# YichengDWu/tinyedm

Hardware: AMD Instinct MI355X
Metric: train imgs/sec CIFAR-10 32x32 bf16 (higher is better)
Workload: dtype bf16; 1 GPU; CIFAR-10 32x32 unconditional EDM2 U-Net (conf/cifar10.yaml, 35.6M params) full training step: diffuse+embed+denoiser fwd/bwd+loss+grad all-reduce+Adam+EMA; per_gpu_batch=128, global_batch=128, parallelism=dp1, conditional=False, step_launch=hipGraph replay, collective=none

## Files before the change

### include/tinyedm_hip.h

```cpp
#ifndef TINYEDM_HIP_H
#define TINYEDM_HIP_H
#ifdef __cplusplus
extern "C" {
#endif

typedef struct ihipStream_t* edm_stream_t;

int edm_version(void);
const char* edm_last_error(void);
int edm_init(int device);
int edm_graph_replay_safe(void);
typedef struct {
  unsigned step, seed_lo, seed_hi, reserved;
  float lr, ema_beta, grad_scale, bc1, bc2sqrt, pad[3];
} edm_step_params;

int edm_conv_igemm(const void* X, const void* Wp, void* Y, const void* R, float alpha, float beta, int B, int H,
                   int W, int Cin, int Cout, int taps, edm_stream_t stream);
int edm_conv_igemm_v2(const void* X, const void* Wp, void* Y, const void* R, float alpha, float beta, int B, int H,
                      int W, int Cin, int Cout, int taps, edm_stream_t stream);
int edm_conv_igemm_v6(const void* X, const void* Wp, void* Y, const void* R, float alpha, float beta, int B, int H,
                      int W, int Cin, int Cout, int taps, edm_stream_t stream);
int edm_conv_igemm_s(const void* X, const void* Wp, void* Y, const void* R, float alpha, float beta, int B, int H,
                     int W, int Cin, int Cout, int taps, edm_stream_t stream);
// ... 82 lines not shown
int edm_attention_fwd(const void* qkv, void* y, int B, int N, int C, int heads, edm_stream_t stream);
int edm_attention_bwd(const void* qkv, const void* y, const void* gy, void* gqkv, int B, int N, int C, int heads,
                      edm_stream_t stream);

int edm_attention_long_supported(int N, int C, int heads);
int edm_attention_long_fwd(const void* qkv, void* y, float* stat, int B, int N, int C, int heads, edm_stream_t stream);
int edm_attention_long_bwd(const void* qkv, const void* y, const void* gy, const float* stat, void* gqkv, float* work,
                           int B, int N, int C, int heads, edm_stream_t stream);

int edm_attention_qkv_supported(int N, int C, int heads);
int edm_attention_qkv_fwd(const void* x, const void* Wqkv, void* y, void* stat, int B, int N, int C, int heads,
                          int heads_per_wg, edm_stream_t stream);
int edm_attention_qkv_bwd(const void* x, const void* y, const void* gout, const void* stat, const void* Wqkv,
                          const void* Wd_out, void* gqkv, float alpha, int B, int N, int C, int heads, int heads_per_wg,
                          edm_stream_t stream);

int edm_pixelnorm_silu_fwd(const void* x, void* xn, void* a, float* dsave, long P, int C, edm_stream_t stream);
int edm_pixelnorm_silu_bwd(const void* xn, const float* dsave, const void* gxn, float gxn_scale, const void* ga,
                           const void* gadd, void* gx, long P, int C, edm_stream_t stream);
int edm_pool_pixelnorm_silu_fwd(const void* x, void* xn, void* a, float* dsave, int B, int Hp, int Wp, int C,
                                edm_stream_t stream);
int edm_pool_pixelnorm_silu_bwd(const void* xn, const float* dsave, const void* gxn, float gxn_scale, const void* ga,
                                const void* gadd, void* gx, int B, int Hp, int Wp, int C, edm_stream_t stream);
int edm_silu_fwd(const void* x, void* a, long n, edm_stream_t stream);
int edm_silu_bwd(const void* x, const void* ga, const void* gextra, float extra_scale, void* gx, long n,
                 edm_stream_t stream);
int edm_axpby(const void* a, float alpha, const void* b, float beta, void* out, long n, edm_stream_t stream);
int edm_mod_silu_drop_fwd(const void* r, const float* lin, long lin_stride, const float* gain, void* a, int B, int HW,
                          int C, float pdrop, unsigned long long seed, unsigned sub, unsigned step, const void* dyn,
                          edm_stream_t stream);
int edm_mod_silu_drop_bwd(const void* r, const float* lin, long lin_stride, const float* gain, const void* ga, void* gr,
                          float* gm, float* glin, long glin_stride, float* ggain, int B, int HW, int C, float pdrop,
                          unsigned long long seed, unsigned sub, unsigned step, const void* dyn, edm_stream_t stream);
int edm_mod_silu_drop_bwd_raw(const void* r, const float* lin, long lin_stride, const float* gain, const void* ga, void* gr,
                              float* gm, long gm_stride, int B, int HW, int C, float pdrop, unsigned long long seed,
                              unsigned sub, unsigned step, const void* dyn, edm_stream_t stream);
int edm_dropout_mask(unsigned char* mask, long n, float pdrop, unsigned long long seed, unsigned sub, unsigned step,
                     edm_stream_t stream);
int edm_pool2(const void* x, void* y, int B, int Hout, int Wout, int C, float scale, edm_stream_t stream);
int edm_up2(const void* x, const void* add, void* y, int B, int Hout, int Wout, int C, float scale, edm_stream_t stream);
int edm_up2_silu(const void* x, void* y, void* a, int B, int Hout, int Wout, int C, edm_stream_t stream);
int edm_reduce_hw(const void* x, long x_stride, const void* y, long y_stride, float* out, int B, int HW, int C,
                  float scale, edm_stream_t stream);
int edm_scalelong_fwd(const float* mean, const float* W1h, const float* W2h, float* gate, float* z1save, int B, int C,
                      int R, edm_stream_t stream);
int edm_scalelong_bwd(const float* mean, const float* W1h, const float* W2h, const float* gate, const float* z1save,
// ... 321 lines not shown
```

### tinyedm_amd/_lib.py

```python
import ctypes
import os

_HERE = os.path.dirname(os.path.abspath(__file__))
LIB_PATH = os.environ.get("EDM_LIB_PATH") or os.path.join(_HERE, "libtinyedm_hip.so")

P, I, L, F = ctypes.c_void_p, ctypes.c_int, ctypes.c_long, ctypes.c_float
U, U64 = ctypes.c_uint, ctypes.c_ulonglong
D = ctypes.c_double

SIGNATURES = {
    "edm_version": [],
    "edm_last_error": [],
    "edm_init": [I],
    "edm_graph_replay_safe": [],
    "edm_pixelnorm_silu_fwd": [P, P, P, P, L, I, P],
    "edm_pixelnorm_silu_bwd": [P, P, P, F, P, P, P, L, I, P],
    "edm_pool_pixelnorm_silu_fwd": [P, P, P, P, I, I, I, I, P],
    "edm_pool_pixelnorm_silu_bwd": [P, P, P, F, P, P, P, I, I, I, I, P],
    "edm_up2_silu": [P, P, P, I, I, I, I, P],
    "edm_silu_fwd": [P, P, L, P],
    "edm_silu_bwd": [P, P, P, F, P, L, P],
    "edm_axpby": [P, F, P, F, P, L, P],
    "edm_mod_silu_drop_fwd": [P, P, L, P, P, I, I, I, F, U64, U, U, P, P],
    "edm_mod_silu_drop_bwd": [P, P, L, P, P, P, P, P, L, P, I, I, I, F, U64, U, U, P, P],
    "edm_mod_silu_drop_bwd_raw": [P, P, L, P, P, P, P, L, I, I, I, F, U64, U, U, P, P],
    "edm_dropout_mask": [P, L, F, U64, U, U, P],
    "edm_pool2": [P, P, I, I, I, I, F, P],
    "edm_up2": [P, P, P, I, I, I, I, F, P],
    "edm_reduce_hw": [P, L, P, L, P, I, I, I, F, P],
    "edm_scalelong_fwd": [P, P, P, P, P, I, I, I, P],
    "edm_scalelong_bwd": [P, P, P, P, P, P, P, P, P, I, I, I, P],
    "edm_skip_gate_fwd": [P, P, P, P, P, P, I, I, I, I, P],
    "edm_skip_gate_bwd": [P, L, I, P, P, P, P, P, P, P, P, P, P, I, I, I, I, P],
    "edm_skip_gate_wgrad_multi": [P, I, P, P, I, P],
    "edm_skip_gate_wgrad_multi_table_bytes": [],
    "edm_skip_gate_fwd_multi": [P, I, P, P, I, P],
    "edm_skip_gate_fwd_multi_table_bytes": [],
    "edm_skip_gate_bwd_multi": [P, I, P, P, I, P],
    "edm_skip_half_bwd_multi": [P, I, P, P, I, P],
    "edm_skip_gate_bwd_multi_table_bytes": [],
    "edm_concat_gate_fwd": [P, P, P, P, P, I, I, I, I, P],
# ... 255 lines not shown
```

### tinyedm_amd/csrc/elementwise.hip

```cpp
#include "common.h"
#include <stdarg.h>
#include <stdio.h>

static thread_local char g_err[512] = "";
extern "C" void edm_set_error(const char* fmt, ...) {
  va_list ap;
  va_start(ap, fmt);
  vsnprintf(g_err, sizeof(g_err), fmt, ap);
  va_end(ap);
}
extern "C" const char* edm_last_error() { return g_err; }
extern "C" int edm_version() { return 1; }

static inline int cdiv(long a, long b) { return (int)((a + b - 1) / b); }
static inline int grid_for(long work, int block, int cap = 256 * 16) {
  long g = (work + block - 1) / block;
  if (g > cap) g = cap;
  if (g < 1) g = 1;
  return (int)g;
}

template <int LPP, bool POOL = false>
__global__ __launch_bounds__(256) void k_pnorm_silu_fwd(const bf16* __restrict__ x, bf16* __restrict__ xn,
                                                          bf16* __restrict__ a, float* __restrict__ dsave, int P,
                                                          int C, int Hp = 0, int Wp = 0) {
// ... 34 lines not shown
      }
    }
    ss = group_sum<LPP>(ss);
    const float d = NORM_EPS + sqrtf(ss) * rsC;
    const float inv = 1.0f / d;
#pragma unroll
    for (int it = 0; it < 2; ++it) {
      const int c8 = lig + it * LPP;
      if (pv && c8 < CL) {
        float o[8], s[8];
#pragma unroll
        for (int i = 0; i < 8; ++i) {
          o[i] = (float)(bf16)(v[it][i] * inv);
          s[i] = mp_silu_b(o[i]);
        }
        store8(xn + p * C + c8 * 8, o);
        store8(a + p * C + c8 * 8, s);
      }
    }
    if (pv && lig == 0) dsave[p] = d;
  }
}

template <int LPP, bool UP = false>
__global__ __launch_bounds__(256) void k_pnorm_silu_bwd(const bf16* __restrict__ xn, const float* __restrict__ dsave,
                                                          const bf16* __restrict__ gxn, float gs,
                                                          const bf16* __restrict__ ga, const bf16* __restrict__ gadd,
                                                          bf16* __restrict__ gx, int P, int C, int Hp = 0, int Wp = 0) {
  constexpr int GPW = 64 / LPP;
  const int lane = threadIdx.x & 63, wave = threadIdx.x >> 6;
  const int lig = lane % LPP, grp = lane / LPP;
  const int CL = C >> 3;
  const long stride = (long)gridDim.x * 4 * GPW;
  for (long p0 = ((long)blockIdx.x * 4 + wave) * GPW; p0 < P; p0 += stride) {
    const long p = p0 + grp;
    const bool pv = p < P;
    float y[2][8], g[2][8];
    float dot = 0.f;
#pragma unroll
    for (int it = 0; it < 2; ++it) {
      const int c8 = lig + it * LPP;
      if (pv && c8 < CL) {
        load8(xn + p * C + c8 * 8, y[it]);
        float t[8];
        if (gxn) {
          load8(gxn + p * C + c8 * 8, t);
#pragma unroll
          for (int i = 0; i < 8; ++i) g[it][i] = gs * t[i];
        } else {
#pragma unroll
          for (int i = 0; i < 8; ++i) g[it][i] = 0.f;
// ... 14 lines not shown
    float inv = 1.0f / d;
#pragma unroll
    for (int it = 0; it < 2; ++it) {
      const int c8 = lig + it * LPP;
      if (pv && c8 < CL) {
        float o[8];
#pragma unroll
        for (int i = 0; i < 8; ++i) o[i] = (g[it][i] - y[it][i] * coef) * inv;
        if constexpr (UP) {
          const int w = (int)(p % Wp);
          const long t2 = p / Wp;
          const int h = (int)(t2 % Hp);
          const long b = t2 / Hp;
          const long e0 = ((b * 2 * Hp + 2 * h) * 2 * Wp + 2 * w) * C + c8 * 8;
          const long row = (long)2 * Wp * C;
#pragma unroll
          for (int i = 0; i < 8; ++i) o[i] = 0.25f * (float)(bf16)o[i];
#pragma unroll
          for (int q = 0; q < 4; ++q) {
            const long e = e0 + (q >> 1) * row + (q & 1) * C;
            float r[8];
#pragma unroll
            for (int i = 0; i < 8; ++i) r[i] = o[i];
            if (gadd) {
              float t[8];
              load8(gadd + e, t);
#pragma unroll
              for (int i = 0; i < 8; ++i) r[i] += t[i];
            }
            store8(gx + e, r);
          }
          continue;
        }
        if (gadd) {
          float t[8];
          load8(gadd + p * C + c8 * 8, t);
#pragma unroll
          for (int i = 0; i < 8; ++i) o[i] += t[i];
        }
        store8(gx + p * C + c8 * 8, o);
      }
    }
  }
}

static int pick_lpp(int C) {
  int cl = C / 8;
  return cl <= 16 ? 16 : (cl <= 32 ? 32 : 64);
}

extern "C" int edm_pixelnorm_silu_fwd(const void* x, void* xn, void* a, float* dsave, long P, int C,
                                      hipStream_t st) {
  EDM_REQUIRE(P > 0 && P < (1L << 31) && C > 0 && C % 8 == 0 && C <= 1024, "pixelnorm_silu_fwd: bad P=%ld C=%d", P, C);
  int lpp = pick_lpp(C);
  int gpw = 64 / lpp;
  int grid = grid_for(P, 4 * gpw);
#define L(N) hipLaunchKernelGGL(k_pnorm_silu_fwd<N>, dim3(grid), dim3(256), 0, st, (const bf16*)x, (bf16*)xn, (bf16*)a, dsave, (int)P, C)
  if (lpp == 16) L(16); else if (lpp == 32) L(32); else L(64);
#undef L
  EDM_CHECK_LAUNCH("pixelnorm_silu_fwd");
  return EDM_OK;
}
// ... 5 lines not shown
  const long P = (long)B * Hp * Wp;
  int lpp = pick_lpp(C);
  int gpw = 64 / lpp;
  int grid = grid_for(P, 4 * gpw);
#define L(N) hipLaunchKernelGGL((k_pnorm_silu_fwd<N, true>), dim3(grid), dim3(256), 0, st, (const bf16*)x, (bf16*)xn, (bf16*)a, dsave, (int)P, C, Hp, Wp)
  if (lpp == 16) L(16); else if (lpp == 32) L(32); else L(64);
#undef L
  EDM_CHECK_LAUNCH("pool_pixelnorm_silu_fwd");
  return EDM_OK;
}
extern "C" int edm_pool_pixelnorm_silu_bwd(const void* xn, const float* dsave, const void* gxn, float gxn_scale,
                                           const void* ga, const void* gadd, void* gx, int B, int Hp, int Wp, int C,
                                           hipStream_t st) {
  EDM_REQUIRE(xn && dsave && gx && B > 0 && Hp > 0 && Wp > 0 && C > 0 && C % 8 == 0 && C <= 1024 &&
                  (long)B * Hp * Wp < (1L << 31), "pool_pixelnorm_silu_bwd: bad args");
  const long P = (long)B * Hp * Wp;
  int lpp = pick_lpp(C);
  int gpw = 64 / lpp;
  int grid = grid_for(P, 4 * gpw);
#define L(N) hipLaunchKernelGGL((k_pnorm_silu_bwd<N, true>), dim3(grid), dim3(256), 0, st, (const bf16*)xn, dsave, (const bf16*)gxn, gxn_scale, (const bf16*)ga, (const bf16*)gadd, (bf16*)gx, (int)P, C, Hp, Wp)
  if (lpp == 16) L(16); else if (lpp == 32) L(32); else L(64);
#undef L
  EDM_CHECK_LAUNCH("pool_pixelnorm_silu_bwd");
  return EDM_OK;
}

extern "C" int edm_pixelnorm_silu_bwd(const void* xn, const float* dsave, const void* gxn, float gxn_scale,
                                      const void* ga, const void* gadd, void* gx, long P, int C, hipStream_t st) {
  EDM_REQUIRE(P > 0 && P < (1L << 31) && C > 0 && C % 8 == 0 && C <= 1024, "pixelnorm_silu_bwd: bad P=%ld C=%d", P, C);
  int lpp = pick_lpp(C);
  int gpw = 64 / lpp;
  int grid = grid_for(P, 4 * gpw);
#define L(N) hipLaunchKernelGGL(k_pnorm_silu_bwd<N>, dim3(grid), dim3(256), 0, st, (const bf16*)xn, dsave, (const bf16*)gxn, gxn_scale, (const bf16*)ga, (const bf16*)gadd, (bf16*)gx, (int)P, C)
  if (lpp == 16) L(16); else if (lpp == 32) L(32); else L(64);
#undef L
  EDM_CHECK_LAUNCH("pixelnorm_silu_bwd");
  return EDM_OK;
}

__global__ void k_silu_fwd(const bf16* __restrict__ x, bf16* __restrict__ a, long n8) {
  for (long i = (long)blockIdx.x * blockDim.x + threadIdx.x; i < n8; i += (long)gridDim.x * blockDim.x) {
    float v[8];
    load8(x + i * 8, v);
#pragma unroll
    for (int j = 0; j < 8; ++j) v[j] = mp_silu_b(v[j]);
    store8(a + i * 8, v);
// ... 1371 lines not shown
```

### tinyedm_amd/networks.py

```python
from __future__ import annotations

import contextlib
import math
import os
from typing import Optional

import numpy as np
import torch
import torch.nn as nn
from torch import Tensor

from . import ops

bf16, f32 = torch.bfloat16, torch.float32


class _Rng:
    seed: int = 42
    step: int = 0
    dyn = None


rng = _Rng()

# ... 81 lines not shown
            if len(pend) >= FIN_GROUP:
                _flush_fin(key)
            _queue_backward_end(w.device)
            return None
        g = ops.wgrad_finish(slabs, w.data, self._taps(), I, perm=self._perm, scale=scale)
        return g.view_as(w)


WGRAD_STREAM = os.environ.get("EDM_WGRAD_STREAM", "1") != "0"
W3_GROUP = max(0, min(ops.W3_MAX_LAYERS, int(os.environ.get("EDM_W3_GROUP", "16"))))
W3_TAIL = max(0, int(os.environ.get("EDM_W3_TAIL", "0")))
_w3_seen = {}
_w3_total = {}
W3_MAXPIX = int(os.environ.get("EDM_W3_MAXPIX", str(1 << 18)))
FIN_GROUP = 40
W1_GROUP = max(0, min(16, int(os.environ.get("EDM_W1_GROUP", "16"))))
_w1_pending = {}
_bwd_end_queued = set()
MOD_DEFER_UNFUSED = os.environ.get("EDM_MOD_DEFER_UNFUSED", "1") != "0"
SG_MULTI = os.environ.get("EDM_SG_MULTI", "1") != "0"
SG_HALVES = os.environ.get("EDM_SG_HALVES", "1") != "0"
SG_BWD_MULTI = os.environ.get("EDM_SG_BWD_MULTI", "1") != "0"
SG_DEFER = os.environ.get("EDM_SG_DEFER", "1") != "0"
_sg_pending = {}
_w3_pending = {}
TAIL_LOWRANK = os.environ.get("EDM_TAIL_LOWRANK", "1") != "0"
_tail_slot = {}
TAIL_FWD = os.environ.get("EDM_TAIL_FWD", "1") != "0"
_tail_fwd_slot = {}
_fin_pending = {}


def _run_on_side(device, fn, tensors=()):
    if WGRAD_STREAM:
        side = ops.side_stream(device)
        side.wait_stream(torch.cuda.current_stream())
        with torch.cuda.stream(side):
            fn()
        for t in tensors:
            t.record_stream(side)
    else:
        fn()


class FusedOptPass:

# ... 63 lines not shown
    dev = items[0][1].device
    args = [(slabs, w.data, w.grad, perm, taps, I, scale, True) for slabs, w, perm, taps, I, scale in items]
    _run_on_side(dev, lambda: ops.wgrad_finish_multi(args), [a[0] for a in args])
    for _, w, *_rest in items:
        w._edm_deferred = False
        for hook in getattr(w, "_edm_hooks", ()):
            hook(w)


def _flush_sg(key):
    items = _sg_pending.pop(key, None)
    if not items:
        return
    outs = ops.skip_gate_wgrad_multi([(ws, mean, R) for _, ws, mean, R in items])
    for (sl, _, _, _), (gw1h, gw2h) in zip(items, outs):
        sl.layer1.finish_grad(gw1h.view(1, 1, *gw1h.shape))
        sl.layer2.finish_grad(gw2h.view(1, 1, *gw2h.shape))


def _backward_end(key):
    _bwd_end_queued.discard(key)
    _tail_slot.pop(key, None)
    _tail_fwd_slot.pop(key, None)
    if key in _w3_seen:
        _w3_total[key] = _w3_seen.pop(key)
    _flush_sg(key)
    _flush_w3(key)
    _flush_fin(key)
    if WGRAD_STREAM:
        torch.cuda.current_stream(key).wait_stream(ops.side_stream(key))


def _queue_backward_end(device):
    key = torch.device(device).index
    if key in _bwd_end_queued:
        return
    try:
        torch.autograd.Variable._execution_engine.queue_callback(lambda: _backward_end(key))
        _bwd_end_queued.add(key)
    except RuntimeError:
        _backward_end(key)


def reset_backward_state():
    _tail_slot.clear()
    _tail_fwd_slot.clear()
    if _bwd_end_queued or _w3_pending or _fin_pending or _w1_pending or _sg_pending:
        _bwd_end_queued.clear()
        for items in _sg_pending.values():
            for sl, *_rest in items:
                sl.layer1.weight._edm_deferred = sl.layer2.weight._edm_deferred = False
        _sg_pending.clear()
        for items in _w1_pending.values():
            for m, _, _, _ in items:
                m.weight._edm_deferred = False
        _w1_pending.clear()
        for items in _fin_pending.values():
            for _, w, *_rest in items:
                w._edm_deferred = False
        _fin_pending.clear()
        for items in _w3_pending.values():
            for m, _, _, _ in items:
                m.weight._edm_deferred = False
        _w3_pending.clear()
        _w3_seen.clear()
        if WGRAD_STREAM:
            for s in ops.side_streams():
                torch.cuda.current_stream(s.device).wait_stream(s)

# ... 608 lines not shown
                gqkv = ops.attention_bwd(qkv, y, gy, mod.num_heads)
        gw_out = _wgrad(mod.out_conv, y, gout, 1, b)
        gx = ops.conv_igemm(gqkv, wd_qkv, 1, residual=gout, alpha=1.0, beta=a)
        gw_qkv = _wgrad(mod.qkv_conv, x, gqkv, 1)
        return gx, gw_qkv, gw_out, None, None, None


class _ResBlockFn(torch.autograd.Function):

    @staticmethod
    def forward(ctx, u, emb, w1x1, w1, w2, wemb, gain, blk, lin_view, glin_view, token, s_pre=None, alias=False,
                gm_view=None, skip=None, w_sl1=None, w_sl2=None, pre=None, dest=None, pool=False, gate_pre=None, tail=0):
        enc = blk.is_encoder
        ctx.set_materialize_grads(False)
        has1 = w1x1 is not None
        taps = 9
        wf1, wd1, _ = blk.conv_3x3_1.packs()
        wf2, wd2, _ = blk.conv_3x3_2.packs()
        batched = lin_view is not None
        weh = None if batched else blk.embed.packs()[2]
        wf11 = wd11 = None
        tail_fwd = False
        ctx.has_skip = skip is not None
        if skip is not None:
            sl = blk.cat_factor
            ctx.sgb = None
            if gate_pre is not None:
                mean, gate, z1, w1h, w2h, ctx.sgb, halves = gate_pre
            else:
                w1h, w2h = sl.layer1.packs()[2], sl.layer2.packs()[2]
                mean, gate, z1 = ops.skip_gate_fwd(skip, w1h, w2h)
            ctx.Ci = u.shape[-1]
            if pre is not None and pre[0].shape[-1] == u.shape[-1] + skip.shape[-1] and pre[0].data_ptr() == u.data_ptr():
                cat, s_pre = pre
                if not (gate_pre is not None and halves == cat.data_ptr()):
                    ops.skip_half_fwd(skip, gate, cat, s_pre)
            else:
                cat, s_pre = ops.concat_gate_fwd(u.contiguous(), skip, gate, True)
            u = cat
            ctx.skip_saved = (skip, mean, gate, z1, w1h, w2h)
        ctx.pool = bool(pool)
        if enc and pool:
            assert not has1
            xres, s, dsave = ops.pool_pixelnorm_silu_fwd(u)
        elif enc:
            x = u
            if has1:
                wf11, wd11, _ = blk.conv_1x1.packs()
                x = ops.conv_igemm(u, wf11, 1)
# ... 108 lines not shown
            ggain = None
            if not deferred and not only:
                for hook in getattr(gp, "_edm_hooks", ()):
                    hook(gp)
        if tfwd is not None:
            gw2 = _wgrad_lowrank(blk.conv_3x3_2, a2, tail[0], tail[1], b, G=tfwd[0])
        elif tail is not None:
            gw2 = _wgrad_lowrank(blk.conv_3x3_2, a2, tail[0], tail[1], b)
        else:
            gw2 = _wgrad(blk.conv_3x3_2, a2, gout, 9, b)
        gwemb = gemb = gtoken = None
        if ctx.batched:
            gtoken = ops.zeros_f32((1,), gout.device) if (ctx.has_token and not only) else None
        elif only:
            pass
        else:
            dweh = ops.linear_wgrad(glin, emb)
            gwemb = blk.embed.finish_grad(dweh.view(1, 1, *dweh.shape))
            gemb = ops.linear_dgrad(glin, weh) if ctx.needs_input_grad[1] else None
        fuse = ops.FUSE_MOD and ops.IGEMM_VERSION == 0 and not enc
        gs = None if fuse else ops.conv_igemm(gr1, wd1, 9)
        gw1 = _wgrad(blk.conv_3x3_1, s, gr1, 9)
        gw11 = None
        if enc and ctx.pool:
            gu = ops.pool_pixelnorm_silu_bwd(xn, dsave, gout, a, gs, gadd=g_alias)
            g_alias = None
        elif enc:
            gx = ops.pixelnorm_silu_bwd(xn, dsave, gout, a, gs, gadd=None if has1 else g_alias)
            if has1:
                gw11 = _wgrad(blk.conv_1x1, u, gx, 1)
                gu = ops.conv_igemm(gx, wd11, 1, residual=g_alias, alpha=1.0, beta=1.0 if g_alias is not None else 0.0)
            else:
                gu = gx
            g_alias = None
        else:
            if tfwd is not None:
                t = ops.conv3x3_silubwd(gr1, wd1, u) if fuse else ops.silu_bwd(u, gs)
                gu, gcs = ops.lowrank_gcat_add(tail[0], tfwd[2], a, t, ctx.Ci if ctx.has_skip else None)
                if has1:
                    gw11 = _wgrad_lowrank(blk.conv_1x1, None, None, tail[1], a, G=tfwd[1])
            elif has1:
                t = ops.conv3x3_silubwd(gr1, wd1, u) if fuse else ops.silu_bwd(u, gs)
                if ctx.has_skip:
                    Ci = ctx.Ci
                    B_, H_, W_, Ct = u.shape
                    gu = torch.empty(B_, H_, W_, Ci, device=u.device, dtype=bf16)
                    gcs = torch.empty(B_, H_, W_, Ct - Ci, device=u.device, dtype=bf16)
                    ops.conv_igemm(gout, wd11, 1, residual=t, alpha=a, beta=1.0, split=(Ci, gu, gcs))
                else:
                    gu = ops.conv_igemm(gout, wd11, 1, residual=t, alpha=a, beta=1.0)
                    gcs = None
                gw11 = _wgrad(blk.conv_1x1, u, gout, 1, a)
            else:
                gu = ops.conv3x3_silubwd(gr1, wd1, u, gout, a) if fuse else ops.silu_bwd(u, gs, gout, a)
                gcs = None
        gskip = gwsl1 = gwsl2 = None
        if ctx.has_skip:
            skip, mean, gate, z1, w1h, w2h = ctx.skip_saved
            Ci = ctx.Ci
            sl = blk.cat_factor
            wsl = (sl.layer1.weight, sl.layer2.weight)
            defer = SG_DEFER and all(w.grad is not None and getattr(w, "_edm_direct", False) for w in wsl)
            sgb = getattr(ctx, "sgb", None)
            queued = False
            if only:
                if gcs is None:
                    gmean, _ws = ops.skip_gate_bwd(gu, Ci, skip, mean, w1h, w2h, gate, z1, defer_wgrad=True)
                    gu, gskip = ops.concat_gate_bwd(gu, gate, gmean, Ci)
                elif defer and sgb is not None and SG_BWD_MULTI:
                    gskip = torch.empty_like(gcs)
                    sgb.pending.append((gcs, skip, w1h, w2h, gate, z1, gskip, sl, mean))
                else:
                    gmean, _ws = ops.skip_gate_bwd(gcs, 0, skip, mean, w1h, w2h, gate, z1, defer_wgrad=True)
                    gskip = ops.skip_half_bwd(gcs, gate, gmean)
            elif gcs is None:
                gmean, *gws = ops.skip_gate_bwd(gu, Ci, skip, mean, w1h, w2h, gate, z1, defer_wgrad=defer)
                gu, gskip = ops.concat_gate_bwd(gu, gate, gmean, Ci)
            elif defer and sgb is not None and SG_BWD_MULTI:
                gskip = torch.empty_like(gcs)
                sgb.pending.append((gcs, skip, w1h, w2h, gate, z1, gskip, sl, mean))
                queued = True
            else:
                gmean, *gws = ops.skip_gate_bwd(gcs, 0, skip, mean, w1h, w2h, gate, z1, defer_wgrad=defer)
                gskip = ops.skip_half_bwd(gcs, gate, gmean)
            if only:
                pass
            elif defer:
                if not queued:
                    _sg_pending.setdefault(wsl[0].device.index, []).append((sl, gws[0], mean, w1h.shape[0]))
                wsl[0]._edm_deferred = wsl[1]._edm_deferred = True
                _queue_backward_end(wsl[0].device)
            else:
                gw1h, gw2h = gws
                gwsl1 = sl.layer1.finish_grad(gw1h.view(1, 1, *gw1h.shape))
                gwsl2 = sl.layer2.finish_grad(gw2h.view(1, 1, *gw2h.shape))
            if sgb is not None:
                sgb.arrived += 1
                if sgb.arrived == sgb.expected:
                    sgb.flush()
        if g_alias is not None:
            gu = ops.axpby(gu, 1.0, g_alias, 1.0)
        return (gu, gemb, gw11, gw1, gw2, gwemb, ggain, None, None, None, gtoken, None, None, None, gskip, gwsl1, gwsl2,
                None, None, None, None, None)


_rng_sub_counter = [0]


class _BlockBase(nn.Module):
    is_encoder = True

    def _common(self, out_channels, embedding_dim, attention, num_heads, dropout_rate):
        self.conv_3x3_2 = Conv2d(out_channels, out_channels, 3)
        self.dropout = nn.Dropout(dropout_rate)
        self.attention = CosineAttention(out_channels, num_heads) if attention else nn.Identity()
        self.embed = Linear(embedding_dim, out_channels)
        self.embed.weight._edm_late = True
        self.gain = nn.Parameter(torch.ones(()))
        self._tail_last = False
# ... 93 lines not shown


def _tag(x: Tensor) -> Tensor:
    x._edm_nhwc = True
    return x


class EncoderBlock(_BlockBase):
    is_encoder = True

    def __init__(self, in_channels: int, out_channels: int, embedding_dim: int, down: bool, attention: bool,
                 num_heads: int = 4, dropout_rate: float = 0.0, add_factor: float = 0.3):
        super().__init__()
        self.dropout_rate = dropout_rate
        self.add_factor = add_factor
        self.resample = DownSample() if down else nn.Identity()
        self.conv_1x1 = Conv2d(in_channels, out_channels, 1) if in_channels != out_channels else nn.Identity()
        self.conv_3x3_1 = Conv2d(out_channels, out_channels, 3)
        self._common(out_channels, embedding_dim, attention, num_heads, dropout_rate)

    def forward(self, input: Tensor, embedding: Tensor, _lin=None, _alias: bool = False, _dest=None):
        x, conv = _as_nhwc(input)
        ualias = None
        emb = None if _lin is not None else _emb32(embedding, x.shape[0])
        if (isinstance(self.resample, DownSample) and FUSE_RESAMPLE and not isinstance(self.conv_1x1, Conv2d)
                and x.shape[-1] <= 1024 and x.shape[1] % 2 == 0 and x.shape[2] % 2 == 0):
            out = self._res(x, emb, _lin, alias=_alias, pool=True, dest=_dest)
            if _alias:
                out, ualias = out
        else:
            if isinstance(self.resample, DownSample):
                if _alias:
                    x, ualias = _ResampleFn.apply(x, False, True)
                else:
                    x = _ResampleFn.apply(x, False)
            if _alias and ualias is None:
                out, ualias = self._res(x, emb, _lin, alias=True, dest=_dest)
            else:
                out = self._res(x, emb, _lin, dest=_dest)
        if conv:
            out = ops.nhwc_bf16_to_nchw(out).to(input.dtype)
        else:
            cat_pre = getattr(out, "_edm_cat", None)
            out = _tag(out)
            if cat_pre is not None:
                out._edm_cat = cat_pre
        return (out, _tag(ualias)) if _alias else out

    def forward_f32(self, x: Tensor, lin: Tensor, want=None):
        pairs = _split_ok(self.conv_3x3_1)
        if (F32_FUSE_OUT and isinstance(self.resample, DownSample) and not isinstance(self.conv_1x1, Conv2d)
                and x.shape[-1] <= 1024):
            xn, s = ops.f32_pool_pixelnorm_silu(x, pairs=pairs)
        else:
            if isinstance(self.resample, DownSample):
                x = ops.f32_pool2(x)
            if isinstance(self.conv_1x1, Conv2d):
                x = _conv_f32(self.conv_1x1, x, 1)
            xn, s = ops.f32_pixelnorm_silu(x, pairs=pairs)
        return _res_f32(self, xn, s, lin, want)


class DecoderBlock(_BlockBase):
    is_encoder = False

    def __init__(self, in_channels: int, out_channels: int, embedding_dim: int, up: bool, attention: bool,
                 num_heads: int = 4, skip_channels: int = 0, dropout_rate: float = 0.0, add_factor: float = 0.3):
        super().__init__()
        self.add_factor = add_factor
# ... 591 lines not shown
        B = noisy.shape[0]
        sig = sigma.detach().float().flatten().contiguous()
        emb = _emb32(embedding, B)

        blocks = self._res_blocks()
        lin_all, glin_all, token, gm_all = _EmbedAllFn.apply(emb, self, *[b.embed.weight for b in blocks])
        lins, off = {}, 0
        for k, b in enumerate(blocks):
            C = b.embed.weight.shape[0]
            lins[b] = (lin_all[:, off:off + C], glin_all[:, off:off + C], token if k == 0 else None,
                       None if gm_all is None else gm_all[:, off:off + C])
            off += C

        link = [] if (torch.is_grad_enabled() and noisy.requires_grad) else None
        x = _ConvInFn.apply(noisy, sig, self.conv_in.weight, self, link)
        skips = []
        dec = list(zip(self.decoder_blocks, self.skip_connections))
        enc = list(self.encoder_blocks)
        for k, block in enumerate(enc):
            dest = None
            if k + 1 == len(enc) and dec and not dec[0][1]:
                dest = self._silu_dest(block, dec[0][0], x, 1, down=isinstance(block.resample, DownSample))
            x, x_in = block(_tag(x), None, _lin=lins[block], _alias=True, _dest=dest)
            skips.append(x_in)
        skips.append(x)
        dests = _decoder_dests_impl(dec, skips, x) if FUSE_CAT and SKIP_GATE_FUSED else {}
        gates = self._decoder_gates(dec, skips, dests) if SG_MULTI else {}
        tail_co = self._tail_fwd_co()
        for i, (block, has_skip) in enumerate(dec):
            skip = skips.pop() if has_skip else None
            dest = dests.get(i)
            if dest is not None:
                pass
            elif i + 1 < len(dec):
                dest = self._silu_dest(block, dec[i + 1][0], x, 2 if isinstance(block.resample, UpSample) else 1)
            xin = _tag(x)
            cat_pre = getattr(x, "_edm_cat", None)
            if cat_pre is not None:
                xin._edm_cat = cat_pre
            last = {"_tail": tail_co} if (tail_co and i + 1 == len(dec)) else {}
            x = block(xin, None, _tag(skip) if has_skip else None, _lin=lins[block], _dest=dest, _gate=gates.get(block), **last)
        D = self._conv_out_of(x, noisy, sig, link)
        if self.training:
            rng.step += 1
        return D.to(noisy_image.dtype)


class _SgbPass:

    def __init__(self, expected: int):
        self.expected, self.arrived, self.pending = expected, 0, []

    def flush(self):
        items, self.pending = self.pending, []
        self.arrived = 0
        if not items:
            return
        by_c = {}
        for it in items:
            by_c.setdefault(it[1].shape[-1], []).append(it)
        halves = []
        for group in by_c.values():
            for k0 in range(0, len(group), 32):
                part = group[k0:k0 + 32]
                res = ops.skip_gate_bwd_multi([(gcs, 0, skip, w1h, w2h, gate, z1) + ((gskip,) if SG_HALVES else ())
                                               for gcs, skip, w1h, w2h, gate, z1, gskip, _, _ in part])
                for (gcs, skip, w1h, w2h, gate, z1, gskip, sl, mean), (gmean, ws) in zip(part, res):
                    if not SG_HALVES:
                        halves.append((gcs, gate, gmean, gskip))
                    if _DGRAD_ONLY[0]:
                        continue
                    _sg_pending.setdefault(sl.layer1.weight.device.index, []).append((sl, ws, mean, w1h.shape[0]))
        for k0 in range(0, len(halves), 32):
            ops.skip_half_bwd_multi(halves[k0:k0 + 32])


def _decoder_dests_impl(dec, skips, x):
    out = {}
    st = list(skips)
    h, w = x.shape[1], x.shape[2]
    for i, (block, has_skip) in enumerate(dec):
        if has_skip:
            st.pop()
        if isinstance(block.resample, UpSample):
            h, w = 2 * h, 2 * w
        if i + 1 < len(dec) and dec[i + 1][1]:
            nxt = dec[i + 1][0]
            if not isinstance(nxt.resample, UpSample) and isinstance(nxt.conv_1x1, Conv2d):
                Ct = block.conv_3x3_2.weight.shape[0] + st[-1].shape[-1]
                out[i] = (torch.empty(x.shape[0], h, w, Ct, device=x.device, dtype=bf16),
                          torch.empty(x.shape[0], h, w, Ct, device=x.device, dtype=bf16))
# ... 49 lines not shown
```

### tinyedm_amd/ops.py

```python
import contextlib
import ctypes
import functools
import math
import os
import types
from typing import NamedTuple, Optional

import numpy as np
import torch

from . import _lib

bf16, f32 = torch.bfloat16, torch.float32

PROFILE = None


class _prof:
    def __init__(self, name, flops, nbytes):
        self.name, self.flops, self.nbytes = name, flops, nbytes

    def __enter__(self):
        if PROFILE is not None:
            self.s = torch.cuda.Event(enable_timing=True)
# ... 281 lines not shown
    return t.shape


def pixelnorm_silu_fwd(x):
    B, H, W, C = _nhwc(x, "x")
    xn, a = torch.empty_like(x), torch.empty_like(x)
    d = torch.empty(B * H * W, device=x.device, dtype=f32)
    _lib.call("edm_pixelnorm_silu_fwd", _p(x), _p(xn), _p(a), _p(d), B * H * W, C, _stream())
    return xn, a, d


def pixelnorm_silu_bwd(xn, d, gxn, gxn_scale, ga, gadd=None):
    B, H, W, C = _nhwc(xn, "xn")
    _chk(d, f32, "d", (B * H * W,))
    if gxn is not None:
        _chk(gxn, bf16, "gxn", xn.shape)
    if ga is not None:
        _chk(ga, bf16, "ga", xn.shape)
    if gadd is not None:
        _chk(gadd, bf16, "gadd", xn.shape)
    gx = torch.empty_like(xn)
    _lib.call("edm_pixelnorm_silu_bwd", _p(xn), _p(d), _p(gxn), float(gxn_scale), _p(ga), _p(gadd), _p(gx), B * H * W, C,
              _stream())
    return gx


def pool_pixelnorm_silu_fwd(x):
    B, H, W, C = _nhwc(x, "x")
    if H % 2 or W % 2 or C > 1024:
        raise ValueError("pool_pixelnorm_silu_fwd: H, W even and C <= 1024 required")
    xn = torch.empty(B, H // 2, W // 2, C, device=x.device, dtype=bf16)
    a = torch.empty_like(xn)
    d = torch.empty(B * (H // 2) * (W // 2), device=x.device, dtype=f32)
    _lib.call("edm_pool_pixelnorm_silu_fwd", _p(x), _p(xn), _p(a), _p(d), B, H // 2, W // 2, C, _stream())
    return xn, a, d


def pool_pixelnorm_silu_bwd(xn, d, gxn, gxn_scale, ga, gadd=None):
    B, H, W, C = _nhwc(xn, "xn")
    _chk(d, f32, "d", (B * H * W,))
    if gxn is not None:
        _chk(gxn, bf16, "gxn", xn.shape)
    if ga is not None:
        _chk(ga, bf16, "ga", xn.shape)
    if gadd is not None:
        _chk(gadd, bf16, "gadd", (B, 2 * H, 2 * W, C))
# ... 3009 lines not shown
```

### tinyedm_amd/vjp.py

```python
from __future__ import annotations

import torch

from . import networks

__all__ = ["input_vjp", "open_input_vjp"]


def _bf16_only(den) -> None:
    if getattr(den, "eval_dtype", "bf16") != "bf16":
        raise ValueError(f"input_vjp: the denoiser evaluates in {den.eval_dtype!r}, a forward-only path; the backward exists "
                         "on the bf16 path: call set_eval_dtype(\"bf16\") (generate: --network_dtype bf16)")


def _check_inputs(x, sigma) -> None:
    if not isinstance(x, torch.Tensor) or not x.dtype.is_floating_point or x.dim() != 4:
        raise ValueError("input_vjp: x must be a floating-point [B, C, H, W] tensor")
    if not x.is_cuda:
        raise ValueError(f"input_vjp: x is on {x.device}; the library's networks run on the GPU only")
    if not isinstance(sigma, torch.Tensor) or sigma.device != x.device:
        raise ValueError(f"input_vjp: sigma must be a tensor on {x.device}")


def _library_parts(model):
# ... 35 lines not shown
            else:
                if not isinstance(labels_or_embedding, torch.Tensor):
                    raise ValueError("input_vjp: a Denoiser takes the embedding tensor as its fourth argument")
                emb = labels_or_embedding
            emb = emb.detach()
        prev, networks._DGRAD_ONLY[0] = networks._DGRAD_ONLY[0], True
        try:
            with torch.enable_grad():
                xr = x.detach().float().contiguous().requires_grad_()
                D = den(xr, sigma.detach(), emb)
        finally:
            networks._DGRAD_ONLY[0] = prev
    finally:
        owner.train(was_training)

    def pullback(cotangent):
        _check_cotangent(cotangent, D)
        prev, networks._DGRAD_ONLY[0] = networks._DGRAD_ONLY[0], True
        try:
            (g,) = torch.autograd.grad(D, xr, cotangent.detach().float().contiguous())
        finally:
            networks._DGRAD_ONLY[0] = prev
            networks._tail_slot.pop(dev, None)
        return g
    return D.detach(), pullback


def _check_cotangent(cotangent, D) -> None:
    if not isinstance(cotangent, torch.Tensor) or not cotangent.dtype.is_floating_point:
        raise ValueError("input_vjp: cotangent must be a floating-point tensor")
    if tuple(cotangent.shape) != tuple(D.shape):
        raise ValueError(f"input_vjp: cotangent must have D's shape {tuple(D.shape)}, got {tuple(cotangent.shape)}")
    if cotangent.device != D.device:
        raise ValueError(f"input_vjp: cotangent is on {cotangent.device}, D on {D.device}")


def input_vjp(model, x, sigma, labels_or_embedding=None, cotangent=None):
    if cotangent is None:
        raise ValueError("input_vjp: cotangent is required (the vector of the vector-Jacobian product)")
    D, pullback = open_input_vjp(model, x, sigma, labels_or_embedding)
    return D, pullback(cotangent)
```

Baseline: 10370 img/s.

## Fold factored skip-gate gradient into encoder pixelnorm-SiLU backward

In the batched skip-gate backward, the dense skip gradient (gcs*gate + gmean/HW) is no longer materialised. The decoder instead records the concat-gradient slice, gate and gmean, and the matching encoder block's pixelnorm-SiLU backward (plain and pooled variants) recomputes that term on the fly while adding it to its output. This removes a full-size bf16 write and read of the skip gradient per skip connection. In exchange it adds cross-block bookkeeping keyed on tensor pointers, an optional bf16 rounding to match the old numerics, and new error paths for when a backward pass ends partway through the decoder.

```diff
diff --git a/include/tinyedm_hip.h b/include/tinyedm_hip.h
--- a/include/tinyedm_hip.h
+++ b/include/tinyedm_hip.h
@@ -128,6 +128,12 @@
                                 edm_stream_t stream);
 int edm_pool_pixelnorm_silu_bwd(const void* xn, const float* dsave, const void* gxn, float gxn_scale, const void* ga,
                                 const void* gadd, void* gx, int B, int Hp, int Wp, int C, edm_stream_t stream);
+int edm_pixelnorm_silu_bwd_fskip(const void* xn, const float* dsave, const void* gxn, float gxn_scale, const void* ga,
+                                 const void* gcat, long gcat_stride, const float* gate, const float* gmean, int HW,
+                                 int round_bf16, void* gx, long P, int C, edm_stream_t stream);
+int edm_pool_pixelnorm_silu_bwd_fskip(const void* xn, const float* dsave, const void* gxn, float gxn_scale, const void* ga,
+                                      const void* gcat, long gcat_stride, const float* gate, const float* gmean, int HW,
+                                      int round_bf16, void* gx, int B, int Hp, int Wp, int C, edm_stream_t stream);
 int edm_silu_fwd(const void* x, void* a, long n, edm_stream_t stream);
 int edm_silu_bwd(const void* x, const void* ga, const void* gextra, float extra_scale, void* gx, long n,
                  edm_stream_t stream);
diff --git a/tinyedm_amd/_lib.py b/tinyedm_amd/_lib.py
--- a/tinyedm_amd/_lib.py
+++ b/tinyedm_amd/_lib.py
@@ -17,6 +17,8 @@
     "edm_pixelnorm_silu_bwd": [P, P, P, F, P, P, P, L, I, P],
     "edm_pool_pixelnorm_silu_fwd": [P, P, P, P, I, I, I, I, P],
     "edm_pool_pixelnorm_silu_bwd": [P, P, P, F, P, P, P, I, I, I, I, P],
+    "edm_pixelnorm_silu_bwd_fskip": [P, P, P, F, P, P, L, P, P, I, I, P, L, I, P],
+    "edm_pool_pixelnorm_silu_bwd_fskip": [P, P, P, F, P, P, L, P, P, I, I, P, I, I, I, I, P],
     "edm_up2_silu": [P, P, P, I, I, I, I, P],
     "edm_silu_fwd": [P, P, L, P],
     "edm_silu_bwd": [P, P, P, F, P, L, P],
diff --git a/tinyedm_amd/csrc/elementwise.hip b/tinyedm_amd/csrc/elementwise.hip
--- a/tinyedm_amd/csrc/elementwise.hip
+++ b/tinyedm_amd/csrc/elementwise.hip
@@ -1,6 +1,7 @@
 #include "common.h"
 #include <stdarg.h>
 #include <stdio.h>
+#include <type_traits>
 
 static thread_local char g_err[512] = "";
 extern "C" void edm_set_error(const char* fmt, ...) {
@@ -81,11 +82,54 @@
   }
 }
 
-template <int LPP, bool UP = false>
+struct FSkip {
+  long gs;
+  const float* gate;
+  const float* gmean;
+  int HW;
+  float inv_hw;
+  int round_bf16;
+};
+template <bool FS, class Fs>
+__device__ __forceinline__ int fskip_sample(long p, const Fs& fs) {
+  if constexpr (FS) return (int)p / fs.HW;
+  else return 0;
+}
+template <bool FS, class Fs>
+__device__ __forceinline__ void fskip_add8(float* o, const bf16* __restrict__ gadd, long pix, long b, long plain_off,
+                                           int c, int C, const Fs& fs) {
+  float t[8];
+  if constexpr (FS) {
+    load8(gadd + pix * fs.gs + c, t);
+    const float4* gp = reinterpret_cast<const float4*>(fs.gate + b * C + c);
+    const float4* mp = reinterpret_cast<const float4*>(fs.gmean + b * C + c);
+    const float4 g0 = gp[0], g1 = gp[1], m0 = mp[0], m1 = mp[1];
+    const float gt[8] = {g0.x, g0.y, g0.z, g0.w, g1.x, g1.y, g1.z, g1.w};
+    const float mn[8] = {m0.x, m0.y, m0.z, m0.w, m1.x, m1.y, m1.z, m1.w};
+#pragma unroll
+    for (int i = 0; i < 8; ++i) t[i] = __builtin_fmaf(t[i], gt[i], mn[i] * fs.inv_hw);
+    if (fs.round_bf16) {
+#pragma unroll
+      for (int i = 0; i < 8; ++i) t[i] = (float)(bf16)t[i];
+    }
+#pragma unroll
+    for (int i = 0; i < 8; ++i) {
+      asm volatile("" : "+v"(o[i]));
+      o[i] += t[i];
+    }
+  } else {
+    load8(gadd + plain_off, t);
+#pragma unroll
+    for (int i = 0; i < 8; ++i) o[i] += t[i];
+  }
+}
+struct NoFSkip {};
+template <int LPP, bool UP = false, bool FS = false>
 __global__ __launch_bounds__(256) void k_pnorm_silu_bwd(const bf16* __restrict__ xn, const float* __restrict__ dsave,
                                                           const bf16* __restrict__ gxn, float gs,
                                                           const bf16* __restrict__ ga, const bf16* __restrict__ gadd,
-                                                          bf16* __restrict__ gx, int P, int C, int Hp = 0, int Wp = 0) {
+                                                          bf16* __restrict__ gx, int P, int C, int Hp = 0, int Wp = 0,
+                                                          std::conditional_t<FS, FSkip, NoFSkip> fs = {}) {
   constexpr int GPW = 64 / LPP;
   const int lane = threadIdx.x & 63, wave = threadIdx.x >> 6;
   const int lig = lane % LPP, grp = lane / LPP;
@@ -146,22 +190,13 @@
             float r[8];
 #pragma unroll
             for (int i = 0; i < 8; ++i) r[i] = o[i];
-            if (gadd) {
-              float t[8];
-              load8(gadd + e, t);
-#pragma unroll
-              for (int i = 0; i < 8; ++i) r[i] += t[i];
-            }
+            if (FS || gadd)
+              fskip_add8<FS>(r, gadd, (b * 2 * Hp + 2 * h + (q >> 1)) * 2 * Wp + 2 * w + (q & 1), b, e, c8 * 8, C, fs);
             store8(gx + e, r);
           }
           continue;
         }
-        if (gadd) {
-          float t[8];
-          load8(gadd + p * C + c8 * 8, t);
-#pragma unroll
-          for (int i = 0; i < 8; ++i) o[i] += t[i];
-        }
+        if (FS || gadd) fskip_add8<FS>(o, gadd, p, fskip_sample<FS>(p, fs), p * C + c8 * 8, c8 * 8, C, fs);
         store8(gx + p * C + c8 * 8, o);
       }
     }
@@ -213,6 +248,57 @@
   if (lpp == 16) L(16); else if (lpp == 32) L(32); else L(64);
 #undef L
   EDM_CHECK_LAUNCH("pool_pixelnorm_silu_bwd");
+  return EDM_OK;
+}
+
+static int fskip_args(const char* who, const void* gcat, long gs, const float* gate, const float* gmean, int HW,
+                      int round_bf16, long pix, int C, FSkip* fs) {
+  EDM_REQUIRE(gcat && gate && gmean, "%s: null pointer", who);
+  EDM_REQUIRE(HW > 0 && pix % HW == 0, "%s: %ld pixels are no whole samples of HW=%d", who, pix, HW);
+  EDM_REQUIRE(gs >= C && gs % 8 == 0 && ((uintptr_t)gcat & 15) == 0, "%s: gcat rows (stride %ld) must be 16-byte aligned", who, gs);
+  EDM_REQUIRE((((uintptr_t)gate | (uintptr_t)gmean) & 15) == 0, "%s: gate / gmean must be 16-byte aligned", who);
+  fs->gs = gs;
+  fs->gate = gate;
+  fs->gmean = gmean;
+  fs->HW = HW;
+  fs->inv_hw = 1.0f / (float)HW;
+  fs->round_bf16 = round_bf16 != 0;
+  return EDM_OK;
+}
+extern "C" int edm_pixelnorm_silu_bwd_fskip(const void* xn, const float* dsave, const void* gxn, float gxn_scale,
+                                            const void* ga, const void* gcat, long gcat_stride, const float* gate,
+                                            const float* gmean, int HW, int round_bf16, void* gx, long P, int C,
+                                            hipStream_t st) {
+  EDM_REQUIRE(xn && dsave && gx && P > 0 && P < (1L << 31) && C > 0 && C % 8 == 0 && C <= 1024,
+              "pixelnorm_silu_bwd_fskip: bad P=%ld C=%d", P, C);
+  FSkip fs;
+  if (int rc = fskip_args("pixelnorm_silu_bwd_fskip", gcat, gcat_stride, gate, gmean, HW, round_bf16, P, C, &fs)) return rc;
+  int lpp = pick_lpp(C);
+  int gpw = 64 / lpp;
+  int grid = grid_for(P, 4 * gpw);
+#define L(N) hipLaunchKernelGGL((k_pnorm_silu_bwd<N, false, true>), dim3(grid), dim3(256), 0, st, (const bf16*)xn, dsave, (const bf16*)gxn, gxn_scale, (const bf16*)ga, (const bf16*)gcat, (bf16*)gx, (int)P, C, 0, 0, fs)
+  if (lpp == 16) L(16); else if (lpp == 32) L(32); else L(64);
+#undef L
+  EDM_CHECK_LAUNCH("pixelnorm_silu_bwd_fskip");
+  return EDM_OK;
+}
+extern "C" int edm_pool_pixelnorm_silu_bwd_fskip(const void* xn, const float* dsave, const void* gxn, float gxn_scale,
+                                                 const void* ga, const void* gcat, long gcat_stride, const float* gate,
+                                                 const float* gmean, int HW, int round_bf16, void* gx, int B, int Hp,
+                                                 int Wp, int C, hipStream_t st) {
+  EDM_REQUIRE(xn && dsave && gx && B > 0 && Hp > 0 && Wp > 0 && C > 0 && C % 8 == 0 && C <= 1024 &&
+                  (long)B * Hp * Wp < (1L << 29), "pool_pixelnorm_silu_bwd_fskip: bad args");
+  EDM_REQUIRE((long)HW == 4L * Hp * Wp, "pool_pixelnorm_silu_bwd_fskip: HW=%d is not the skip's 4 Hp Wp", HW);
+  const long P = (long)B * Hp * Wp;
+  FSkip fs;
+  if (int rc = fskip_args("pool_pixelnorm_silu_bwd_fskip", gcat, gcat_stride, gate, gmean, HW, round_bf16, 4 * P, C, &fs)) return rc;
+  int lpp = pick_lpp(C);
+  int gpw = 64 / lpp;
+  int grid = grid_for(P, 4 * gpw);
+#define L(N) hipLaunchKernelGGL((k_pnorm_silu_bwd<N, true, true>), dim3(grid), dim3(256), 0, st, (const bf16*)xn, dsave, (const bf16*)gxn, gxn_scale, (const bf16*)ga, (const bf16*)gcat, (bf16*)gx, (int)P, C, Hp, Wp, fs)
+  if (lpp == 16) L(16); else if (lpp == 32) L(32); else L(64);
+#undef L
+  EDM_CHECK_LAUNCH("pool_pixelnorm_silu_bwd_fskip");
   return EDM_OK;
 }
 
diff --git a/tinyedm_amd/networks.py b/tinyedm_amd/networks.py
--- a/tinyedm_amd/networks.py
+++ b/tinyedm_amd/networks.py
@@ -127,6 +127,10 @@
 SG_HALVES = os.environ.get("EDM_SG_HALVES", "1") != "0"
 SG_BWD_MULTI = os.environ.get("EDM_SG_BWD_MULTI", "1") != "0"
 SG_DEFER = os.environ.get("EDM_SG_DEFER", "1") != "0"
+SG_FACTORED = os.environ.get("EDM_SG_FACTORED", "1") != "0"
+SG_FACTORED_ROUND = os.environ.get("EDM_SG_FACTORED", "1") != "2"
+_fskip_slot = {}
+_sgb_active = {}
 _sg_pending = {}
 _w3_pending = {}
 TAIL_LOWRANK = os.environ.get("EDM_TAIL_LOWRANK", "1") != "0"
@@ -236,6 +240,8 @@
     _bwd_end_queued.discard(key)
     _tail_slot.pop(key, None)
     _tail_fwd_slot.pop(key, None)
+    _fskip_slot.pop(key, None)
+    stale = [p.reset() for p in _sgb_active.pop(key, ())]
     if key in _w3_seen:
         _w3_total[key] = _w3_seen.pop(key)
     _flush_sg(key)
@@ -243,6 +249,10 @@
     _flush_fin(key)
     if WGRAD_STREAM:
         torch.cuda.current_stream(key).wait_stream(ops.side_stream(key))
+    if any(stale):
+        raise RuntimeError("tinyedm_amd: the backward pass ended before the gate backward of every U-Net skip had run (it "
+                           "stopped inside the decoder): the skip gradients of this pass are uninitialised and the gates' "
+                           "weight gradients were not reduced.  EDM_SG_BWD_MULTI=0 runs each gate's backward in its block.")
 
 
 def _queue_backward_end(device):
@@ -259,6 +269,11 @@
 def reset_backward_state():
     _tail_slot.clear()
     _tail_fwd_slot.clear()
+    _fskip_slot.clear()
+    for passes in _sgb_active.values():
+        for p in passes:
+            p.reset()
+    _sgb_active.clear()
     if _bwd_end_queued or _w3_pending or _fin_pending or _w1_pending or _sg_pending:
         _bwd_end_queued.clear()
         for items in _sg_pending.values():
@@ -913,9 +928,11 @@
         wf11 = wd11 = None
         tail_fwd = False
         ctx.has_skip = skip is not None
+        ctx.u_key = (u.data_ptr(), tuple(u.shape)) if (enc and alias and w1x1 is None) else None
         if skip is not None:
             sl = blk.cat_factor
             ctx.sgb = None
+            ctx.fskip_ok = SG_FACTORED and getattr(skip, "_edm_fskip", False)
             if gate_pre is not None:
                 mean, gate, z1, w1h, w2h, ctx.sgb, halves = gate_pre
             else:
@@ -1070,7 +1087,17 @@
         gs = None if fuse else ops.conv_igemm(gr1, wd1, 9)
         gw1 = _wgrad(blk.conv_3x3_1, s, gr1, 9)
         gw11 = None
-        if enc and ctx.pool:
+        fskip = None
+        if enc and ctx.u_key is not None:
+            fskip = _fskip_slot.get(gout.device.index, {}).pop(ctx.u_key, None)
+            if fskip is not None and (g_alias is not None or fskip[3] is None):
+                raise RuntimeError("tinyedm_amd: a factored skip gradient reached its encoder block " +
+                                   ("beside a dense one" if g_alias is not None else "before the gate backward had run"))
+        if fskip is not None and ctx.pool:
+            gu = ops.pool_pixelnorm_silu_bwd_fskip(xn, dsave, gout, a, gs, fskip, round_bf16=SG_FACTORED_ROUND)
+        elif fskip is not None:
+            gu = ops.pixelnorm_silu_bwd_fskip(xn, dsave, gout, a, gs, fskip, round_bf16=SG_FACTORED_ROUND)
+        elif enc and ctx.pool:
             gu = ops.pool_pixelnorm_silu_bwd(xn, dsave, gout, a, gs, gadd=g_alias)
             g_alias = None
         elif enc:
@@ -1117,7 +1144,7 @@
                     gu, gskip = ops.concat_gate_bwd(gu, gate, gmean, Ci)
                 elif defer and sgb is not None and SG_BWD_MULTI:
                     gskip = torch.empty_like(gcs)
-                    sgb.pending.append((gcs, skip, w1h, w2h, gate, z1, gskip, sl, mean))
+                    sgb.pending.append((gcs, skip, w1h, w2h, gate, z1, gskip, sl, mean, None))
                 else:
                     gmean, _ws = ops.skip_gate_bwd(gcs, 0, skip, mean, w1h, w2h, gate, z1, defer_wgrad=True)
                     gskip = ops.skip_half_bwd(gcs, gate, gmean)
@@ -1125,8 +1152,14 @@
                 gmean, *gws = ops.skip_gate_bwd(gu, Ci, skip, mean, w1h, w2h, gate, z1, defer_wgrad=defer)
                 gu, gskip = ops.concat_gate_bwd(gu, gate, gmean, Ci)
             elif defer and sgb is not None and SG_BWD_MULTI:
-                gskip = torch.empty_like(gcs)
-                sgb.pending.append((gcs, skip, w1h, w2h, gate, z1, gskip, sl, mean))
+                rec = None
+                if (ctx.fskip_ok and SG_HALVES and ctx.needs_input_grad[14] and not skip.retains_grad
+                        and not skip._backward_hooks and gcs.is_contiguous()):
+                    rec = [gcs, gcs.shape[-1], gate, None, gcs.shape[1] * gcs.shape[2]]
+                    _fskip_slot.setdefault(gcs.device.index, {})[(skip.data_ptr(), tuple(skip.shape))] = rec
+                else:
+                    gskip = torch.empty_like(gcs)
+                sgb.pending.append((gcs, skip, w1h, w2h, gate, z1, gskip, sl, mean, rec))
                 queued = True
             else:
                 gmean, *gws = ops.skip_gate_bwd(gcs, 0, skip, mean, w1h, w2h, gate, z1, defer_wgrad=defer)
@@ -1143,6 +1176,9 @@
                 gwsl1 = sl.layer1.finish_grad(gw1h.view(1, 1, *gw1h.shape))
                 gwsl2 = sl.layer2.finish_grad(gw2h.view(1, 1, *gw2h.shape))
             if sgb is not None:
+                active = _sgb_active.setdefault(gout.device.index, [])
+                if not any(p is sgb for p in active):
+                    active.append(sgb)
                 sgb.arrived += 1
                 if sgb.arrived == sgb.expected:
                     sgb.flush()
@@ -1282,12 +1318,14 @@
     def forward(self, input: Tensor, embedding: Tensor, _lin=None, _alias: bool = False, _dest=None):
         x, conv = _as_nhwc(input)
         ualias = None
+        from_res = False
         emb = None if _lin is not None else _emb32(embedding, x.shape[0])
         if (isinstance(self.resample, DownSample) and FUSE_RESAMPLE and not isinstance(self.conv_1x1, Conv2d)
                 and x.shape[-1] <= 1024 and x.shape[1] % 2 == 0 and x.shape[2] % 2 == 0):
             out = self._res(x, emb, _lin, alias=_alias, pool=True, dest=_dest)
             if _alias:
                 out, ualias = out
+                from_res = True
         else:
             if isinstance(self.resample, DownSample):
                 if _alias:
@@ -1296,6 +1334,7 @@
                     x = _ResampleFn.apply(x, False)
             if _alias and ualias is None:
                 out, ualias = self._res(x, emb, _lin, alias=True, dest=_dest)
+                from_res = True
             else:
                 out = self._res(x, emb, _lin, dest=_dest)
         if conv:
@@ -1305,6 +1344,8 @@
             out = _tag(out)
             if cat_pre is not None:
                 out._edm_cat = cat_pre
+        if _alias and from_res and not isinstance(self.conv_1x1, Conv2d):
+            ualias._edm_alias_res = True
         return (out, _tag(ualias)) if _alias else out
 
     def forward_f32(self, x: Tensor, lin: Tensor, want=None):
@@ -1942,6 +1983,8 @@
             if k + 1 == len(enc) and dec and not dec[0][1]:
                 dest = self._silu_dest(block, dec[0][0], x, 1, down=isinstance(block.resample, DownSample))
             x, x_in = block(_tag(x), None, _lin=lins[block], _alias=True, _dest=dest)
+            if SG_FACTORED and getattr(x_in, "_edm_alias_res", False):
+                x_in._edm_fskip = True
             skips.append(x_in)
         skips.append(x)
         dests = _decoder_dests_impl(dec, skips, x) if FUSE_CAT and SKIP_GATE_FUSED else {}
@@ -1971,6 +2014,10 @@
     def __init__(self, expected: int):
         self.expected, self.arrived, self.pending = expected, 0, []
 
+    def reset(self) -> bool:
+        stale, self.arrived, self.pending = bool(self.pending), 0, []
+        return stale
+
     def flush(self):
         items, self.pending = self.pending, []
         self.arrived = 0
@@ -1983,10 +2030,13 @@
         for group in by_c.values():
             for k0 in range(0, len(group), 32):
                 part = group[k0:k0 + 32]
-                res = ops.skip_gate_bwd_multi([(gcs, 0, skip, w1h, w2h, gate, z1) + ((gskip,) if SG_HALVES else ())
-                                               for gcs, skip, w1h, w2h, gate, z1, gskip, _, _ in part])
-                for (gcs, skip, w1h, w2h, gate, z1, gskip, sl, mean), (gmean, ws) in zip(part, res):
-                    if not SG_HALVES:
+                res = ops.skip_gate_bwd_multi([(gcs, 0, skip, w1h, w2h, gate, z1)
+                                               + ((gskip,) if SG_HALVES and gskip is not None else ())
+                                               for gcs, skip, w1h, w2h, gate, z1, gskip, _, _, _ in part])
+                for (gcs, skip, w1h, w2h, gate, z1, gskip, sl, mean, rec), (gmean, ws) in zip(part, res):
+                    if rec is not None:
+                        rec[3] = gmean
+                    elif not SG_HALVES:
                         halves.append((gcs, gate, gmean, gskip))
                     if _DGRAD_ONLY[0]:
                         continue
diff --git a/tinyedm_amd/ops.py b/tinyedm_amd/ops.py
--- a/tinyedm_amd/ops.py
+++ b/tinyedm_amd/ops.py
@@ -327,6 +327,49 @@
     gx = torch.empty_like(xn)
     _lib.call("edm_pixelnorm_silu_bwd", _p(xn), _p(d), _p(gxn), float(gxn_scale), _p(ga), _p(gadd), _p(gx), B * H * W, C,
               _stream())
+    return gx
+
+
+def _fskip_args(fskip, B, H, W, C):
+    gcat, gs, gate, gmean, HW = fskip[:5]
+    if not isinstance(gcat, torch.Tensor) or not gcat.is_cuda or gcat.dtype != bf16:
+        raise TypeError("fskip gcat: expected a bf16 CUDA/HIP tensor")
+    _chk(gate, f32, "fskip gate", (B, C))
+    _chk(gmean, f32, "fskip gmean", (B, C))
+    gs = int(gs)
+    want = (H * W * gs, W * gs, gs, 1)
+    if (tuple(gcat.shape) != (B, H, W, C) or gs < C or int(HW) != H * W
+            or any(n > 1 and st != w for n, st, w in zip(gcat.shape, gcat.stride(), want))):
+        raise ValueError(f"fskip: gcat {tuple(gcat.shape)} / strides {gcat.stride()} is no (B, H, W, C) = {(B, H, W, C)} tensor "
+                         f"with pixel rows of {gs} elements, or HW = {HW} is not H * W")
+    return gcat.data_ptr(), gs, gate.data_ptr(), gmean.data_ptr(), int(HW)
+
+
+def pixelnorm_silu_bwd_fskip(xn, d, gxn, gxn_scale, ga, fskip, round_bf16=False):
+    B, H, W, C = _nhwc(xn, "xn")
+    _chk(d, f32, "d", (B * H * W,))
+    if gxn is not None:
+        _chk(gxn, bf16, "gxn", xn.shape)
+    if ga is not None:
+        _chk(ga, bf16, "ga", xn.shape)
+    fs = _fskip_args(fskip, B, H, W, C)
+    gx = torch.empty_like(xn)
+    _lib.call("edm_pixelnorm_silu_bwd_fskip", _p(xn), _p(d), _p(gxn), float(gxn_scale), _p(ga), *fs, int(bool(round_bf16)),
+              _p(gx), B * H * W, C, _stream())
+    return gx
+
+
+def pool_pixelnorm_silu_bwd_fskip(xn, d, gxn, gxn_scale, ga, fskip, round_bf16=False):
+    B, H, W, C = _nhwc(xn, "xn")
+    _chk(d, f32, "d", (B * H * W,))
+    if gxn is not None:
+        _chk(gxn, bf16, "gxn", xn.shape)
+    if ga is not None:
+        _chk(ga, bf16, "ga", xn.shape)
+    fs = _fskip_args(fskip, B, 2 * H, 2 * W, C)
+    gx = torch.empty(B, 2 * H, 2 * W, C, device=xn.device, dtype=bf16)
+    _lib.call("edm_pool_pixelnorm_silu_bwd_fskip", _p(xn), _p(d), _p(gxn), float(gxn_scale), _p(ga), *fs,
+              int(bool(round_bf16)), _p(gx), B, H, W, C, _stream())
     return gx
 
 
diff --git a/tinyedm_amd/vjp.py b/tinyedm_amd/vjp.py
--- a/tinyedm_amd/vjp.py
+++ b/tinyedm_amd/vjp.py
@@ -81,6 +81,8 @@
         finally:
             networks._DGRAD_ONLY[0] = prev
             networks._tail_slot.pop(dev, None)
+            for sgb in networks._sgb_active.pop(dev, ()):
+                sgb.reset()
         return g
     return D.detach(), pullback
 
```

Measured after the change: 10440 img/s, median of 6. About the same (+0.6%).
